# Black-Phoenix/CUDA-SfM

Hardware: AMD Instinct MI355X
Metric: RANSAC E-matrix hypotheses/sec (8-point, fused scoring), inlier-mask parity vs CPU oracle (higher is better)
Workload: dtype f32

## Files before the change

### cuda-sfm_amd/csrc/prefilter_lds.hpp

```cpp
#pragma once
#include "prefilter_record.hpp"

namespace sfm {

constexpr int kPfTileMax = 1024;
constexpr int kPfWaves = 16;
constexpr int kPfRing = 128;

constexpr int kPfERow = 10;
constexpr int kPfPassRows = 32, kPfPairRows = 64;
constexpr int pf_wave_bytes(int rows) { return rows * kPfERow * 4 + rows * 4; }
template <int RULE> struct PfLds {
    static constexpr int kFragsPerBlock = RULE == kPfRuleG ? 3 : 2;
    static constexpr int kBlockBytes = kFragsPerBlock * 64 * 16;
    static constexpr int kFrag = 0;
    static constexpr int kTileMax = kPfTileMax;
    int staged, pts, ring, wave, next, lut, bytes;
    __host__ __device__ explicit PfLds(int tile, int ring_entries = kPfRing, int entry_bytes = 8, int rows = RULE == kPfRuleG ? kPfPassRows : kPfPairRows)
    {
        staged = (tile + 63) & ~63;
        pts = kFrag + (staged / 32) * kBlockBytes;
        ring = pts + staged * 16;
        ring = (ring + ring_entries * entry_bytes - 1) & ~(ring_entries * entry_bytes - 1);
        wave = ring + kPfWaves * ring_entries * entry_bytes;
        next = wave + kPfWaves * pf_wave_bytes(rows);
        lut = next + 16;
        bytes = lut + 32;
    }
};
static_assert(kPfRing * 8 == 1024, "ring slots are addressed with (offset & 1023) | base");

static inline int pf_tile_points(int ld, int tmax)
{
    const int ntiles = (ld + tmax - 1) / tmax;
    const int t = ((ld + ntiles - 1) / ntiles + 31) & ~31;
    return t < 32 ? 32 : t;
}

constexpr unsigned long long kPfSumCountsMin = 1ull << 21;
static inline bool pf_sums_counts_at(unsigned count, int ld, int tile)
{
    return (unsigned long long)count * (unsigned long long)((ld + tile - 1) / tile) >= kPfSumCountsMin;
}

constexpr unsigned long long kPfPairPassesMin = 1ull << 22;
static inline bool pf_pairs_passes_at(unsigned count, int ld, int tile)
{
    return (unsigned long long)count * (unsigned long long)((ld + tile - 1) / tile) >= kPfPairPassesMin;
}

}
```

### cuda-sfm_amd/csrc/prefilter_math.hpp

```cpp
#pragma once
#include "device_math.hpp"

namespace sfm {

constexpr int kPfSlots = 32;
constexpr int kPfSlotsT = 16;
constexpr float kPfRho = 0.125f;
constexpr float kPfFeatScale = 16.0f;
constexpr float kPfPadValue = 256.0f;

struct PfScales { int a; float sigE, sigF, sig2a, inv_sig2a; };

SFM_HD bool prefilter_scales(float thr, PfScales &sc)
{
    if (!(thr >= 1e-9f && thr <= 1e-2f)) return false;
    int e = 0;
    (void)frexpf(1.0f / (32.0f * thr), &e);
    const int a = (e - 1) >> 1;
    sc.a = a;
    sc.sigE = ldexpf(1.0f, a - 4);
    sc.sigF = kPfFeatScale;
    sc.sig2a = ldexpf(1.0f, 2 * a);
    sc.inv_sig2a = ldexpf(1.0f, -2 * a);
    return true;
// ... 357 lines not shown

SFM_HD bool prefilter_band_reject(float nt)
{
    return ((f32_bits(nt) >> 30) & 1u) != 0u;
}

SFM_HD bool prefilter_band_pack_reject(float nt)
{
    return fabsf(nt) >= kPfBandPackSwitch;
}

SFM_HD constexpr uint32_t pf_pack_code(int b)
{
    const int bitpos = 31 - b, odd = bitpos & 1, p = bitpos - odd;
    const int reg = (p % 6 == 4) ? 0 : (p % 6 == 2) ? 1 : 2;
    const int f = (32 * (reg + 3 * odd) + p - 4) / 6;
    const int j = f >> 1, st = f & 1;
    return (uint32_t)((j & 3) + 8 * (j >> 2)) | ((uint32_t)st << 5);
}

SFM_HD constexpr uint32_t pf_pack_code_closed(int b)
{
    const uint32_t f = ((5u * ((uint32_t)b >> 1) + 15u) & 15u) | ((~(uint32_t)b & 1u) << 4);
    return ((f >> 1) & 3u) | (f & 24u) | ((f & 1u) << 5);
}
constexpr bool pf_pack_code_closed_ok()
{
    for (int b = 0; b < 32; ++b)
        if (pf_pack_code_closed(b) != pf_pack_code(b)) return false;
    return true;
}
static_assert(pf_pack_code_closed_ok(), "pf_pack_code_closed: the closed form is not the table's permutation");

SFM_HD constexpr uint32_t pf_pack_field_local(int p)
{
    return (uint32_t)(p % 6 == 4 ? p / 6 : p % 6 == 2 ? p / 6 + 5 : p / 6 + 10);
}
SFM_HD constexpr unsigned long long pf_pack_table()
{
    unsigned long long t = 0ull;
    for (int i = 0; i < 16; ++i) t |= (unsigned long long)pf_pack_field_local(30 - 2 * i) << (4 * i);
    return t;
}
SFM_HD uint32_t pf_pack_field(int b)
{
    constexpr unsigned long long kTable = pf_pack_table();
    const uint32_t local = (uint32_t)(kTable >> (((uint32_t)b << 1) & 60u)) & 15u;
    return local + ((~(uint32_t)b & 1u) << 4);
}

SFM_HD void prefilter_transposed(const float e[9], float et[9])
{
    et[0] = e[0]; et[1] = e[3]; et[2] = e[6];
    et[3] = e[1]; et[4] = e[4]; et[5] = e[7];
    et[6] = e[2]; et[7] = e[5]; et[8] = e[8];
}

SFM_HD uint32_t pf_cell_key_side(int ix, int iy, int side)
{
    const uint32_t k = pf_cell_key(ix, iy);
    return side ? ((k ^ 0x2AAAAAAAu) | 1u) : k;
}

}
```

### cuda-sfm_amd/csrc/ransac_prefilter.hip

```cpp
#include "ransac_device.hpp"
#include "block_ops.hpp"
#include "prefilter_math.hpp"
#include "prefilter_record.hpp"
#include "prefilter_lds.hpp"

namespace sfm {

typedef float f16v __attribute__((ext_vector_type(16)));


__device__ constexpr int kPfESlot[9] = { 2, 6, 1, 3, 5, 7, 0, 4, 8 };
__device__ __forceinline__ uint32_t shift_in_reject(uint32_t rejected, float nt, float G)
{
    return __builtin_amdgcn_alignbit(rejected, __float_as_uint(fmaf(-nt, nt, G)), 31);
}

__device__ __forceinline__ uint32_t scan16(const f16v &nt, const f16v &G)
{
    uint32_t rejected = 0u;
#pragma unroll
    for (int r = 0; r < 16; ++r) rejected = shift_in_reject(rejected, nt[r], G[r]);
    return rejected;
}

// ... 65 lines not shown

template <int RULE>
__device__ __forceinline__ void mfma_step(const PfFrags &a, const PfFrags &b, f16v &G, f16v &nt)
{
    const f16v z = {};
    nt = __builtin_amdgcn_mfma_f32_32x32x16_f16(a.n0, b.n0, z, 0, 0, 0);
    if (RULE == kPfRuleG) G = __builtin_amdgcn_mfma_f32_32x32x16_f16(a.t, b.t, z, 0, 0, 0);
    nt = __builtin_amdgcn_mfma_f32_32x32x16_f16(a.n1, b.n1, nt, 0, 0, 0);
}

#define PF_SCHED_STEP()                                                 \
    do {                                                                \
        if (RULE != kPfRuleG) {                                         \
            __builtin_amdgcn_sched_group_barrier(0x008, 1, 0);          \
            __builtin_amdgcn_sched_group_barrier(0x002, 8, 0);          \
            __builtin_amdgcn_sched_group_barrier(0x008, 1, 0);          \
            __builtin_amdgcn_sched_group_barrier(0x002, 8, 0);          \
        } else {                                                        \
            __builtin_amdgcn_sched_group_barrier(0x008, 1, 0);          \
            __builtin_amdgcn_sched_group_barrier(0x002, 11, 0);         \
            __builtin_amdgcn_sched_group_barrier(0x008, 1, 0);          \
            __builtin_amdgcn_sched_group_barrier(0x002, 11, 0);         \
            __builtin_amdgcn_sched_group_barrier(0x008, 1, 0);          \
            __builtin_amdgcn_sched_group_barrier(0x002, 11, 0);         \
        }                                                               \
    } while (0)

constexpr int kPfVarTickets = 1;
constexpr int kPfVarDrainLocal = 2;
constexpr int kPfVarClosedDecode = 4;
constexpr int kPfVarAnswerEpilogue = 8;
constexpr int kPfVarDrainK1 = 16, kPfVarDrainK7 = 32;
constexpr int kPfVarSinglePass = 64;

constexpr int pf_score_waves_per_simd(int var, int rule, int fl2, int pipe, int wide, int prio)
{
    if (var == 0 && rule == kPfRuleBandTile && !fl2 && !pipe && !wide && !prio) return 4;
    return ((var & kPfVarTickets) == 0 && (rule == kPfRuleBandTile || rule == kPfRuleBandPack) && !fl2 && !pipe && !wide && !prio) ? 5 : 4;
}

template <int W, int VAR = 0, int RULE = kPfRuleBandTile, int FL2 = 0, int PIPE = 0, int WIDE = 0, int PRIO = 0>
__global__ __launch_bounds__(W * 64, pf_score_waves_per_simd(VAR, RULE, FL2, PIPE, WIDE, PRIO))
void ransac_score_prefilter(const float *__restrict__ X0, const float *__restrict__ X1, int ld, int n,
                            const float *__restrict__ Ecand, const PfRecord *__restrict__ recs, uint32_t h0, uint32_t count, float thr,
                            int dynamic, int tile,
                            int *__restrict__ counts, uint32_t *__restrict__ tick,
                            unsigned long long *best_key, unsigned long long *best_key2, unsigned long long *__restrict__ clk,
                            const unsigned long long *__restrict__ bound_word, const uint32_t *__restrict__ tile_boxes)
{
    extern __shared__ __attribute__((aligned(16))) unsigned char smem[];
    const int lane = threadIdx.x & 63;
    const int wave = __builtin_amdgcn_readfirstlane(threadIdx.x >> 6);
    const bool probe = clk && blockIdx.x == 0 && blockIdx.y == 0 && threadIdx.x == 0;
    unsigned long long c0 = 0, w0 = 0;
    if (clk && blockIdx.x == 0 && blockIdx.y == 0 && wave == 0) { c0 = clock64(); w0 = wall_clock64(); }
#if SFM_AB
    const uint32_t trace_blk = blockIdx.y * gridDim.x + blockIdx.x;
    unsigned long long *trace = (clk && trace_blk < (uint32_t)kTraceBlocks) ? clk + 8 + (size_t)trace_blk * kTraceWords : nullptr;
    if (trace && threadIdx.x == 0) {
        trace[0] = wall_clock64();
        trace[2] = ((unsigned long long)__builtin_amdgcn_s_getreg((20 << 0) | (0 << 6) | (31 << 11)) << 32) |
                   (unsigned long long)__builtin_amdgcn_s_getreg((4 << 0) | (0 << 6) | (31 << 11));
        trace[3] = ((unsigned long long)blockIdx.y << 32) | blockIdx.x;
    }
#define PF_PHASE(k) do { if (probe1) clk[k] = wall_clock64() - w0; } while (0)
#else
#define PF_PHASE(k) do { } while (0)
#endif
    const int half = lane >> 5, row = lane & 31;
    uint32_t npass = (count + (uint32_t)kPfGroup - 1u) / (uint32_t)kPfGroup;
    const uint32_t nstatic = gridDim.x * (uint32_t)W;
    using LT = PfLds<RULE>;
    constexpr bool kBand = RULE != kPfRuleG, kTile = RULE == kPfRuleBandTile, kPack = RULE == kPfRuleBandPack || kTile;
    static_assert(!(FL2 && kPack) && !((VAR & kPfVarTickets) && kPack), "the recorded variants were built on the v_alignbit scan");
    constexpr bool kTail9 = kPack && W == 16 && !FL2 && !PIPE && !WIDE && !PRIO && !(VAR & kPfVarTickets);
    static_assert(kTail9 || (VAR & ~kPfVarTickets) == 0, "the pass-tail switches belong to the product's two rules");
    static_assert(!(VAR & kPfVarSinglePass) || (kTile && VAR == kPfVarSinglePass), "single passes: the per-tile rule's summing instance");
    constexpr bool kPair = kTile && kTail9 && VAR == 0;
    constexpr int kRows = kPair ? kPfPairRows : kPfPassRows, kUnit = kRows;
    constexpr int kDrainMore = !kTail9 ? 0 : (VAR & kPfVarDrainK1) ? 1 : (VAR & kPfVarDrainK7) ? 7 : (VAR & kPfVarDrainLocal) ? 3 : 0;
    constexpr bool kDecodeTable = !(kTail9 && (VAR & kPfVarClosedDecode));
    constexpr bool kSumCounts = kTail9 && !(VAR & kPfVarAnswerEpilogue);
    constexpr int kRing = FL2 ? 256 : kPfRing;
    constexpr int kEnt = WIDE ? 16 : 8;
    static_assert(!WIDE || (kPack && !PIPE && !FL2), "wide entries: the packed scan's plain loop only");
    if (kPair) npass = (npass + 1u) >> 1;
    const LT L(tile, kRing, kEnt, kRows);
    float *etab = reinterpret_cast<float *>(smem + L.wave + wave * pf_wave_bytes(kRows));
    int *cnt = reinterpret_cast<int *>(etab + kRows * kPfERow);

    PfFrags afrag = {};
    h8 bfrag_n0 = {}, bfrag_n1 = {};
    uint32_t key0 = 0u;
    float rec_dn = 0.0f, rec_lin = 0.0f;
    float e_row[9] = {};
    auto fetch_pass = [&](uint32_t pass, PfFrags &af, uint32_t &k0, float (&e)[9], float &dn, float &lin) {
        const uint32_t hf = pass * (uint32_t)kUnit;
        const uint32_t h = hf + (uint32_t)min(kPair ? lane : row, (int)min((uint32_t)kUnit, count - hf) - 1);
        if (kTile) {
            const float *src = Ecand + 9 * (size_t)h;
#pragma unroll
            for (int k = 0; k < 9; ++k) e[k] = src[k];
            const uint4 rec = reinterpret_cast<const uint4 *>(recs)[h];
            k0 = rec.x; dn = __uint_as_float(rec.y); lin = __uint_as_float(rec.z);
            return;
        }
        const uint4 *r = reinterpret_cast<const uint4 *>(recs + h) + 2 * half;
        const uint4 r0 = r[0], r1 = r[1];
        if (kBand) pf_band_record_expand(r0, r1, half, af.n0, af.n1, k0);
        else pf_record_expand(r0, r1, half, af.n0, af.n1, af.t, k0);
        if (half == 0) {
            const float *src = Ecand + 9 * (size_t)h;
#pragma unroll
            for (int k = 0; k < 9; ++k) e[k] = src[k];
        }
    };
    auto install_rows = [&](const float (&e)[9]) {
        if (kPair || half == 0) {
            const int r = kPair ? lane : row;
#pragma unroll
            for (int k = 0; k < 9; ++k) etab[kRows * k + r] = e[kPfESlot[k]];
            cnt[r] = 0;
        }
    };
    uint32_t ps = blockIdx.x * (uint32_t)W + (uint32_t)wave;
    bool have = ps < npass;
    if (have) { fetch_pass(ps, afrag, key0, e_row, rec_dn, rec_lin); install_rows(e_row); }

    SFM_PHASE("stage_tile");
    uint32_t *next_idx = reinterpret_cast<uint32_t *>(smem + L.next);
    if (threadIdx.x == 0) *next_idx = (uint32_t)W;
    if (kPack && kDecodeTable && threadIdx.x < 32) smem[L.lut + threadIdx.x] = (unsigned char)pf_pack_code((int)threadIdx.x);
    float pf_B = 0.0f;
    uint32_t bw[8] = {};
    uint32_t bw_lane = 0u;
    if (kTile) {
        pf_B = __uint_as_float((uint32_t)(__hip_atomic_load(reinterpret_cast<const uint32_t *>(bound_word), __ATOMIC_RELAXED, __HIP_MEMORY_SCOPE_AGENT)));
        bw_lane = __hip_atomic_load(tile_boxes + 8 * blockIdx.y + (lane & 7), __ATOMIC_RELAXED, __HIP_MEMORY_SCOPE_AGENT);
    }
    __syncthreads();
    const int tile_first = blockIdx.y * tile;
    for (int t = threadIdx.x; t < L.staged; t += W * 64) {
        const int p = tile_first + t;
        float u = 0.f, v = 0.f, x = 0.f, y = 0.f;
        const bool real = p < n && t < tile;
        if (kTile) {
            if (real) {
                const float4 q4 = reinterpret_cast<const float4 *>(X0)[p];
                u = q4.x; v = q4.y; x = q4.z; y = q4.w;
            }
        } else
        if (real) { u = X0[p]; v = X0[(size_t)ld + p]; x = X1[p]; y = X1[(size_t)ld + p]; }
        _Float16 bn[kPfSlots], bt[kPfSlotsT];
        prefilter_point_slots(u, v, x, y, real, bn, bt);
        reinterpret_cast<float4 *>(smem + L.pts)[t] = real ? make_float4(x, u, y, v) : make_float4(NAN, NAN, NAN, NAN);
        const int pb = t >> 5, col = t & 31;
        unsigned char *blk = smem + LT::kFrag + pb * LT::kBlockBytes;
#pragma unroll
        for (int ks = 0; ks < 2; ++ks)
#pragma unroll
            for (int hh = 0; hh < 2; ++hh) {
                h8 c;
#pragma unroll
                for (int j = 0; j < 8; ++j) c[j] = bn[ks * 16 + hh * 8 + j];
// ... 30 lines not shown
            bfrag_n0 = __builtin_bit_cast(h8, ya); bfrag_n1 = __builtin_bit_cast(h8, yb);
        } else
        pf_tile_operands(e, fl, dn, lin, thr_l, B_l, tbox, half_l, afrag.n0, afrag.n1);
    };
    if (kTile) {
#pragma unroll
        for (int k = 0; k < 8; ++k) bw[k] = (uint32_t)__builtin_amdgcn_readlane((int)bw_lane, k);
        pf_B = uniform(pf_B);
        tbox = pf_box_from_bits(bw, pf_B);
        tbox = PfBox{ uniform(tbox.xlo), uniform(tbox.xhi), uniform(tbox.ylo), uniform(tbox.yhi), uniform(tbox.ulo), uniform(tbox.uhi), uniform(tbox.vlo), uniform(tbox.vhi) };
        if (have) build_operands(e_row, key0, rec_dn, rec_lin);
    }
#if SFM_AB
    if (probe) clk[2] = wall_clock64() - w0;
#endif
    const int npb = (min(tile, ld - tile_first) + 31) >> 5;
    const int npp = (npb + 1) >> 1;
    const float4 *pts = reinterpret_cast<const float4 *>(smem + L.pts);
    lds_cf *etab_l = (lds_cf *)etab;
    lds_i *cnt_l = (lds_i *)cnt;
    lds_cu8 *lut_l = (lds_cu8 *)(smem + L.lut);
    const uint32_t ring_base = (uint32_t)(size_t)(__attribute__((address_space(3))) unsigned char *)(smem + L.ring) + (uint32_t)wave * (uint32_t)(kRing * kEnt);
    uint32_t ring_mask = (uint32_t)(kRing * kEnt - 1);
    asm("" : "+v"(ring_mask));
    auto ring_at = [&](uint32_t index8) {
        return (lds_u2 *)((__attribute__((address_space(3))) unsigned char *)0 + ((index8 & ring_mask) | ring_base));
    };
    auto ring_at16 = [&](uint32_t index16) {
        return (lds_u4 *)((__attribute__((address_space(3))) unsigned char *)0 + ((index16 & ring_mask) | ring_base));
    };
    lds_ch8 *frag_lane = (lds_ch8 *)(smem + LT::kFrag) + lane;
    const ThrBand band = make_band(thr);
    uint32_t passes_done = 0;

    while (have) {
        SFM_PHASE("pass_begin");
        const uint32_t h_first = ps * (uint32_t)kUnit;
        const int nvalid_unit = (int)min((uint32_t)kUnit, count - h_first);
        int nvalid = min(nvalid_unit, kPfGroup), hoff = 0;
        const int nscan = (kPair && nvalid_unit > kPfGroup) ? 2 : 1;
#if SFM_AB
        const bool probe1 = probe && passes_done == 0u;
#endif
        uint32_t ps_next = ps + nstatic;
        if (dynamic) {
            uint32_t got = 0u;
            if (lane == 0) got = atomicAdd(next_idx, 1u);
            got = (uint32_t)__builtin_amdgcn_readfirstlane((int)got);
            ps_next = (got / (uint32_t)W) * nstatic + blockIdx.x * (uint32_t)W + (got % (uint32_t)W);
        }
        const unsigned long long scan_rows = __ballot(key0 != 0u);
        int head = 0, nq = 0;
        auto patch_zero_divisor_rows = [&](int sc) {
            uint32_t todo = kPair ? (uint32_t)(sc ? scan_rows >> 32 : scan_rows) : ((uint32_t)scan_rows | (uint32_t)(scan_rows >> 32));
            uint32_t survive = 0u;
            while (todo) {
                const int r = __builtin_ctz(todo) + hoff;
                todo &= todo - 1u;
                const float se[6] = { etab[6 * kRows + r], etab[2 * kRows + r], etab[r], etab[3 * kRows + r], etab[7 * kRows + r], etab[4 * kRows + r] };
                bool z = false;
                for (int j = 0; j < L.staged / 64; ++j) {
                    const float4 q = pts[j * 64 + lane];
                    z = z || prefilter_zero_divisor(se, q.x, q.z);
                }
                if (__ballot(z) != 0ull) survive |= 1u << (r - hoff);
            }
            if (survive != 0u && ((survive >> row) & 1u)) {
                const h8 zero = {};
                afrag.n0 = zero; afrag.n1 = zero; afrag.t = zero;
                if (half) { afrag.n1[3] = (_Float16)1.0f; afrag.t[7] = (_Float16)0.0009765625f; }
            }
        };

        const uint32_t lane_tag = (uint32_t)(size_t)(lds_cf4 *)pts + (uint32_t)(row * 16) + (uint32_t)(half * 4);
        auto decide_first = [&](uint32_t &rest, uint32_t tag) {
            const int b = __builtin_clz(rest);
            rest &= ~(0x80000000u >> b);
            int hl, sub;
            if (kPack) {
                const uint32_t code = kDecodeTable ? (uint32_t)lut_l[b] : pf_pack_code_closed(b);
                hl = (int)(code & 31u) + (int)(tag & 4u); sub = (int)(code >> 5);
            } else {
                const int r = kBand ? b >> 1 : b & 15;
                sub = kBand ? b & 1 : b >> 4;
                hl = r + (r & 12) + (int)(tag & 4u);
            }
            if (hl < nvalid) {
                const f4v q = *(lds_cf4 *)((__attribute__((address_space(3))) const unsigned char *)0 + ((tag & ~15u) + ((uint32_t)sub << 9)));
                lds_cf *e = etab_l + hl + hoff;
                const v2f p0 = { e[0], e[kRows] }, p1 = { e[2 * kRows], e[3 * kRows] }, p2 = { e[4 * kRows], e[5 * kRows] }, p3 = { e[6 * kRows], e[7 * kRows] };
                const float e8 = e[8 * kRows];
                if (pf_exact_inlier(p0, p1, p2, p3, e8, v2f{ q.x, q.y }, v2f{ q.z, q.w }, band))
                    __hip_atomic_fetch_add(cnt_l + hl + hoff, 1, __ATOMIC_RELAXED, __HIP_MEMORY_SCOPE_WORKGROUP);
            }
        };
        auto flush = [&](int m, auto more_c) {
            constexpr int kMore = decltype(more_c)::value;
            uint32_t rest = 0, tag = 0;
            if (PRIO == 2) __builtin_amdgcn_s_setprio(2);
            if (lane < m) {
                const u2v ent = *ring_at(((uint32_t)head + (uint32_t)lane) * 8u);
                tag = ent.y;
                rest = ent.x;
                decide_first(rest, tag);
                if constexpr (kMore > 0) {
#pragma unroll 1
                    for (int it = 0; it < kMore && rest != 0u; ++it) decide_first(rest, tag);
                }
            }
            const unsigned long long more = __ballot(rest != 0u);
            if (more) {
                const int slot = __builtin_amdgcn_mbcnt_hi((uint32_t)(more >> 32), __builtin_amdgcn_mbcnt_lo((uint32_t)more, 0u));
                if (rest) *ring_at(((uint32_t)(head + nq) + (uint32_t)slot) * 8u) = u2v{ rest, tag };
            }
            head = (head + m) & (kRing - 1);
            nq += __builtin_popcountll(more) - m;
            if (PRIO == 2) __builtin_amdgcn_s_setprio(0);
        };
        constexpr std::integral_constant<int, 0> kInLoop{};
        constexpr std::integral_constant<int, kDrainMore> kDrain{};
        auto flush_w = [&](int m) {
            uint32_t ra = 0, rb = 0, tag = 0;
            if (lane < m) {
                const u4v ent = *ring_at16(((uint32_t)head + (uint32_t)lane) * 16u);
                tag = ent.z;
                const bool second = ent.x == 0u;
// ... 22 lines not shown
        };
        auto flush2 = [&]() {
            const u2v entA = *ring_at(((uint32_t)head + (uint32_t)lane) * 8u), entB = *ring_at(((uint32_t)head + 64u + (uint32_t)lane) * 8u);
            const int bA = __builtin_clz(entA.x), bB = __builtin_clz(entB.x);
            const uint32_t restA = entA.x & ~(0x80000000u >> bA), restB = entB.x & ~(0x80000000u >> bB);
            const int rA = bA >> 1, rB = bB >> 1;
            const int hlA = rA + (rA & 12) + (int)(entA.y & 4u), hlB = rB + (rB & 12) + (int)(entB.y & 4u);
            const int hcA = min(hlA, nvalid - 1), hcB = min(hlB, nvalid - 1);
            const f4v qA = *(lds_cf4 *)((__attribute__((address_space(3))) const unsigned char *)0 + ((entA.y & ~15u) + ((uint32_t)(bA & 1) << 9)));
            const f4v qB = *(lds_cf4 *)((__attribute__((address_space(3))) const unsigned char *)0 + ((entB.y & ~15u) + ((uint32_t)(bB & 1) << 9)));
            lds_cf *eA = etab_l + hcA, *eB = etab_l + hcB;
            const v2f a0 = { eA[0], eA[32] }, a1 = { eA[64], eA[96] }, a2 = { eA[128], eA[160] }, a3 = { eA[192], eA[224] };
            const float a8 = eA[256];
            const v2f b0 = { eB[0], eB[32] }, b1 = { eB[64], eB[96] }, b2 = { eB[128], eB[160] }, b3 = { eB[192], eB[224] };
            const float b8 = eB[256];
            const bool inA = pf_exact_inlier(a0, a1, a2, a3, a8, v2f{ qA.x, qA.y }, v2f{ qA.z, qA.w }, band);
            const bool inB = pf_exact_inlier(b0, b1, b2, b3, b8, v2f{ qB.x, qB.y }, v2f{ qB.z, qB.w }, band);
            if (inA && hlA < nvalid) __hip_atomic_fetch_add(cnt_l + hlA, 1, __ATOMIC_RELAXED, __HIP_MEMORY_SCOPE_WORKGROUP);
            if (inB && hlB < nvalid) __hip_atomic_fetch_add(cnt_l + hlB, 1, __ATOMIC_RELAXED, __HIP_MEMORY_SCOPE_WORKGROUP);
            const unsigned long long moreA = __ballot(restA != 0u), moreB = __ballot(restB != 0u);
            if (moreA | moreB) {
                const int nA = __builtin_popcountll(moreA);
                const int slotA = __builtin_amdgcn_mbcnt_hi((uint32_t)(moreA >> 32), __builtin_amdgcn_mbcnt_lo((uint32_t)moreA, 0u));
                const int slotB = nA + __builtin_amdgcn_mbcnt_hi((uint32_t)(moreB >> 32), __builtin_amdgcn_mbcnt_lo((uint32_t)moreB, 0u));
                if (restA) *ring_at(((uint32_t)(head + nq) + (uint32_t)slotA) * 8u) = u2v{ restA, entA.y };
                if (restB) *ring_at(((uint32_t)(head + nq) + (uint32_t)slotB) * 8u) = u2v{ restB, entB.y };
            }
            head = (head + 128) & (kRing - 1);
            nq += __builtin_popcountll(moreA) + __builtin_popcountll(moreB) - 128;
        };

        for (int sc = 0; ; ++sc) {
        patch_zero_divisor_rows(sc);
        PF_PHASE(3);
        if constexpr (kPack && PIPE) {
        PfFrags fa = load_point_frags<RULE>(frag_lane, 0), fb = load_point_frags<RULE>(frag_lane, 1);
        lds_ch8 *fp = frag_lane + 2 * (LT::kBlockBytes / 16);
        const f16v zero16 = {};
        f16v a0, a1, b0, b1;
        a0 = __builtin_amdgcn_mfma_f32_32x32x16_f16(afrag.n0, fa.n0, zero16, 0, 0, 0);
        a1 = __builtin_amdgcn_mfma_f32_32x32x16_f16(afrag.n0, fb.n0, zero16, 0, 0, 0);
        a0 = __builtin_amdgcn_mfma_f32_32x32x16_f16(afrag.n1, fa.n1, a0, 0, 0, 0);
        a1 = __builtin_amdgcn_mfma_f32_32x32x16_f16(afrag.n1, fb.n1, a1, 0, 0, 0);
        fa = load_point_frags<RULE>(fp, 0);
        fb = load_point_frags<RULE>(fp, 1);
        fp += 2 * (LT::kBlockBytes / 16);
        auto phase = [&](const f16v &c0, const f16v &c1, f16v &m0, f16v &m1, int pp) {
            SFM_PHASE("scan_two_steps");
            __builtin_amdgcn_sched_barrier(0);
            m0 = __builtin_amdgcn_mfma_f32_32x32x16_f16(afrag.n0, fa.n0, zero16, 0, 0, 0);
            __builtin_amdgcn_sched_barrier(0);
            const u6v d = __builtin_amdgcn_cvt_scalef32_2xpk16_bf6_f32(c0, c1, 1.0f);
            __builtin_amdgcn_sched_barrier(0);
            m1 = __builtin_amdgcn_mfma_f32_32x32x16_f16(afrag.n0, fb.n0, zero16, 0, 0, 0);
            __builtin_amdgcn_sched_barrier(0);
            const uint32_t rej32 = pack_reject_bits(d);
            __builtin_amdgcn_sched_barrier(0);
            m0 = __builtin_amdgcn_mfma_f32_32x32x16_f16(afrag.n1, fa.n1, m0, 0, 0, 0);
            __builtin_amdgcn_sched_barrier(0);
            const bool mine = rej32 != 0xFFFFFFFFu;
            const unsigned long long any = __ballot(mine);
            __builtin_amdgcn_sched_barrier(0);
            m1 = __builtin_amdgcn_mfma_f32_32x32x16_f16(afrag.n1, fb.n1, m1, 0, 0, 0);
            __builtin_amdgcn_sched_barrier(0);
            fa = load_point_frags<RULE>(fp, 0);
            fb = load_point_frags<RULE>(fp, 1);
            fp += 2 * (LT::kBlockBytes / 16);
// ... 67 lines not shown
        mfma_step<RULE>(afrag, fa, g0, n0);
        lds_ch8 *fp = frag_lane + 2 * (LT::kBlockBytes / 16);
        for (int pp = 0; pp < npp; ++pp) {
            SFM_PHASE("scan_two_steps");
            fa = load_point_frags<RULE>(fp, 0);
            __builtin_amdgcn_sched_barrier(0);
            mfma_step<RULE>(afrag, fb, g1, n1);
            const uint32_t rej_first = kBand ? scan16_band(n0) : scan16(n0, g0);
            PF_SCHED_STEP();
            __builtin_amdgcn_sched_barrier(0);
            fb = load_point_frags<RULE>(fp, 1);
            fp += 2 * (LT::kBlockBytes / 16);
            __builtin_amdgcn_sched_barrier(0);
            mfma_step<RULE>(afrag, fa, g0, n0);
            const uint32_t rej_second = kBand ? scan16_band(n1) : scan16(n1, g1);
            PF_SCHED_STEP();
            __builtin_amdgcn_sched_barrier(0);
            const uint32_t rej32 = kBand ? (((rej_first << 1) & 0xAAAAAAAAu) | (rej_second & 0x55555555u))
                                                       : ((rej_first << 16) | rej_second);
            const bool mine = rej32 != 0xFFFFFFFFu;
            const unsigned long long any = __ballot(mine);
            SFM_PHASE("append_and_inloop_flush");
            if (any) {
                if (FL2) { while (nq >= 128) flush2(); }
                else
                while (nq >= 64) flush(64, kInLoop);
                const int slot = __builtin_amdgcn_mbcnt_hi((uint32_t)(any >> 32), __builtin_amdgcn_mbcnt_lo((uint32_t)any, 0u));
                if (mine) *ring_at(((uint32_t)(head + nq) + (uint32_t)slot) * 8u) = u2v{ ~rej32, lane_tag + ((uint32_t)pp << 10) };
                nq += __builtin_popcountll(any);
            }
        }
        }
        if (sc + 1 >= nscan) break;
        while (nq > 0) flush(min(nq, 64), kDrain);
        afrag.n0 = bfrag_n0; afrag.n1 = bfrag_n1;
        hoff = kPfGroup; nvalid = nvalid_unit - kPfGroup;
        }
        PF_PHASE(4);
        SFM_PHASE("pass_end_fetch_next");
        const bool have_next = ps_next < npass;
        PfFrags afrag_next = afrag;
        uint32_t key0n = 0u;
        float e_next[9] = {}, dn_next = 0.0f, lin_next = 0.0f;
        if (have_next) fetch_pass(ps_next, afrag_next, key0n, e_next, dn_next, lin_next);
        SFM_PHASE("drain_flush");
        if (FL2) { while (nq >= 128) flush2(); }
        if (WIDE) { while (nq > 0) flush_w(min(nq, 64)); }
        while (nq > 0) flush(min(nq, 64), kDrain);
        SFM_PHASE("epilogue");
        PF_PHASE(7);
        if (VAR & kPfVarTickets) {
        if (lane < nvalid) {
            const int c = cnt[lane];
            if (c) atomicAdd(&counts[h_first + lane], c);
        }
        asm volatile("s_waitcnt vmcnt(0)" ::: "memory");
        uint32_t t = 0;
        if (lane == 0) t = atomicAdd(&tick[ps], 1u);
        t = __builtin_amdgcn_readfirstlane(t);
        if (t == gridDim.y - 1) {
            unsigned long long k = 0;
            if (lane < nvalid) {
                const int c = __hip_atomic_load(&counts[h_first + lane], __ATOMIC_RELAXED, __HIP_MEMORY_SCOPE_AGENT);
                k = pack_key((uint32_t)c, h0 + h_first + (uint32_t)lane);
            }
            k = wave_max(k);
            if (lane == 0 && k) {
// ... 21 lines not shown
        }
        const int nvalid_done = nvalid;
        const uint32_t h_done = h_first;
        if (have_next) {
            if (kTile) build_operands(e_next, key0n, dn_next, lin_next);
            else { afrag = afrag_next; key0 = key0n; }
            install_rows(e_next);
        }
        unsigned long long k = 0;
        if (lane < nvalid_done && (uint32_t)(old >> 32) == gridDim.y - 1u) {
            const uint32_t total = (uint32_t)old + c_mine;
            counts[h_done + lane] = (int)total;
            k = pack_key(total, h0 + h_done + (uint32_t)lane);
        }
        if (__ballot(k != 0ull) != 0ull) {
            k = wave_max(k);
            if (lane == 0 && k > __hip_atomic_load(best_key, __ATOMIC_RELAXED, __HIP_MEMORY_SCOPE_AGENT)) {
                atomicMax(best_key, k);
                if (best_key2) atomicMax(best_key2, k);
            }
        }
        }
        PF_PHASE(5);
        ++passes_done;
        have = have_next;
        if (have_next) {
            ps = ps_next;
            if (VAR & kPfVarTickets) { afrag = afrag_next; key0 = key0n; install_rows(e_next); }
        }
    }
    SFM_PHASE("kernel_end");
    if (probe) { clk[6] = passes_done; clk[0] = clock64() - c0; clk[1] = wall_clock64() - w0; }
#if SFM_AB
    if (trace && lane == 0) {
        const unsigned long long tend = wall_clock64();
        trace[4 + wave] = tend;
        if (wave == 0) trace[1] = tend;
    }
#endif
}

constexpr int kPfBuckets = 1024 + 2;
constexpr int kPfBucketBlock = 256;

__device__ __forceinline__ int pf_bucket_of(const float4 q, float B)
{
    const float big = fmaxf(fmaxf(fabsf(q.x), fabsf(q.y)), fmaxf(fabsf(q.z), fabsf(q.w)));
    if (!(big <= 48.0f) || q.x != q.x || q.y != q.y || q.z != q.z || q.w != q.w) return kPfBuckets - 2;
    return (int)(pf_morton_key(q.x, q.y, -B, B, -B, B) >> 20);
}

__global__ __launch_bounds__(1024)
void pf_bucket_scan_kernel(uint32_t *__restrict__ hist, int nblocks, uint32_t *__restrict__ base, uint32_t *__restrict__ boxes, int nbox_words)
{
    for (int k = threadIdx.x; k < nbox_words; k += blockDim.x) boxes[k] = pf_order_bits(-INFINITY);
    __shared__ uint32_t total[kPfBuckets + 1024];
    for (int b = threadIdx.x; b < kPfBuckets; b += blockDim.x) {
        uint32_t run = 0u;
        for (int k = 0; k < nblocks; ++k) {
            const uint32_t c = hist[(size_t)k * kPfBuckets + b];
            hist[(size_t)k * kPfBuckets + b] = run;
            run += c;
        }
        total[b] = run;
    }
    __syncthreads();
// ... 346 lines not shown
constexpr uint64_t kPfOrderFirstCallPairs = 1ull << 33;
int prefilter_pick_rule(sfm_pair *pair, const sfm_ransac_params &p, uint32_t count)
{
    int rule = pf_rule_switch(p);
    if (rule < 0) {
        const bool ordered = pair->sorted_epoch == pair->bound_epoch && pair->d_pts4s != nullptr;
        const bool first = pair->pf_seen_epoch != pair->bound_epoch;
        rule = (!ordered && first && (uint64_t)count * (uint64_t)pair->ld < kPfOrderFirstCallPairs) ? kPfRuleBandPack : kPfRuleBandTile;
    }
    pair->pf_seen_epoch = pair->bound_epoch;
    pair->pf_rule = rule;
    return rule;
}

bool prefilter_usable(const sfm_pair *pair, const sfm_ransac_params &p, uint32_t count)
{
    PfScales sc;
    return pair->state.unit_z && pair->state.have_bound && count >= 16384u && (uint64_t)count * (uint64_t)pair->ld >= (1ull << 27) && prefilter_scales(p.threshold, sc);
}

static int pf_tile_of(const sfm_pair *pair, const sfm_ransac_params &p)
{
    if (SFM_SW(p, 1) == 7 && pair->pf_rule == kPfRuleBand) return pf_tile_points(pair->ld, 1536);
    return pf_tile_points(pair->ld, kPfTileMax);
}

int prefilter_tile_points(const sfm_pair *pair, const sfm_ransac_params &p) { return pf_tile_of(pair, p); }

static int pf_tail_var(const sfm_pair *pair, const sfm_ransac_params &p, uint32_t count)
{
    const bool large = pf_sums_counts_at(count, pair->ld, pf_tile_of(pair, p));
    if (SFM_SW(p, 1) == 19) return 0;
    if (SFM_SW(p, 1) == 20) return pair->pf_rule == kPfRuleBandTile ? kPfVarSinglePass : 0;
    if (pair->pf_rule == kPfRuleBandTile && SFM_SW(p, 1) == 16) return kPfVarDrainK1;
    if (pair->pf_rule == kPfRuleBandTile && SFM_SW(p, 1) == 17) return kPfVarDrainK7;
    int var = 0;
    const bool lab = SFM_SW(p, 3) >= 8 && SFM_SW(p, 3) < 16;
    if (lab && (SFM_SW(p, 3) & 1)) var |= kPfVarDrainLocal;
    if (lab && (SFM_SW(p, 3) & 2)) var |= kPfVarClosedDecode;
    const bool sum = (lab && (SFM_SW(p, 3) & 4)) ? false : (large || (SFM_SW(p, 1) >= 16 && SFM_SW(p, 1) <= 18));
    if (!sum) var |= kPfVarAnswerEpilogue;
    if (var == 0 && pair->pf_rule == kPfRuleBandTile && !pf_pairs_passes_at(count, pair->ld, pf_tile_of(pair, p))) var = kPfVarSinglePass;
    return var;
}

bool prefilter_sums_counts(const sfm_pair *pair, const sfm_ransac_params &p, uint32_t count)
{
    const bool product_rule = pair->pf_rule == kPfRuleBandTile || pair->pf_rule == kPfRuleBandPack;
    const bool variant = SFM_SW(p, 1) == 5 || (SFM_SW(p, 1) >= 11 && SFM_SW(p, 1) <= 15);
    return product_rule && !variant && !(pf_tail_var(pair, p, count) & kPfVarAnswerEpilogue);
}

int launch_score_prefilter(sfm_pair *pair, ShardSlot &s, hipStream_t stream, const sfm_ransac_params &p, uint32_t h0, uint32_t count, unsigned long long *key2)
{
    sfm_ctx *ctx = pair->ctx;
    PfScales sc;
    if (!prefilter_scales(p.threshold, sc)) { set_error("threshold %g outside the pre-filter's range", (double)p.threshold); return SFM_E_INVALID; }
    const int waves = (SFM_SW(p, 1) == 5 || SFM_SW(p, 1) == 12) ? 12 : kPfWaves;
    const int tile = pf_tile_of(pair, p);
    const int ntiles = (pair->ld + tile - 1) / tile;
    const uint32_t npass = (count + (uint32_t)kPfGroup - 1u) / (uint32_t)kPfGroup;
    const int rule = pair->pf_rule;
    const int tail_var = pf_tail_var(pair, p, count);
    const bool wide = rule == kPfRuleBandTile && SFM_SW(p, 1) == 13;
    const bool paired_units = rule == kPfRuleBandTile && tail_var == 0 && waves == kPfWaves && !wide && SFM_SW(p, 1) != 14 && SFM_SW(p, 1) != 15;
    const uint32_t nunits = paired_units ? (npass + 1u) / 2u : npass;
    const uint32_t iters = (nunits + (uint32_t)waves - 1) / (uint32_t)waves;
    uint32_t cols = (uint32_t)ctx->num_cus / (uint32_t)ntiles;
    if (SFM_SW(p, 2) > 0) cols = (uint32_t)SFM_SW(p, 2);
    if (cols > iters) cols = iters;
    if (cols < 1) cols = 1;
    const int dynamic = SFM_SW(p, 1) == 2 ? 0 : 1;
    const int var = SFM_SW(p, 3) >= 16 ? SFM_SW(p, 3) - 16 : 0;
    const bool fl2 = rule == kPfRuleBand && waves == kPfWaves && SFM_SW(p, 1) == 9;
    const int lds_bytes = wide ? PfLds<kPfRuleBand>(tile, kPfRing, 16, kPfPassRows).bytes : fl2 ? PfLds<kPfRuleBand>(tile, 256, 8, kPfPassRows).bytes
                        : rule != kPfRuleG ? PfLds<kPfRuleBand>(tile, kPfRing, 8, paired_units ? kPfPairRows : kPfPassRows).bytes : PfLds<kPfRuleG>(tile).bytes;
    if (lds_bytes > 160 * 1024) { set_error("pre-filter tile of %d points needs %d bytes of LDS", tile, lds_bytes); return SFM_E_INVALID; }
    auto launch = [&](auto kernel) -> int {
        const int rc_lds = allow_big_lds(ctx, reinterpret_cast<const void *>(kernel));
        if (rc_lds != SFM_OK) return rc_lds;
        const float *x0 = rule == kPfRuleBandTile ? reinterpret_cast<const float *>(pair->d_pts4s) : pair->d_X[0];
        hipLaunchKernelGGL(kernel, dim3(cols, ntiles), dim3(waves * 64), lds_bytes, stream,
                           x0, pair->d_X[1], pair->ld, pair->n, s.Ecand, reinterpret_cast<const PfRecord *>(s.pf), h0, count, p.threshold,
                           dynamic, tile, s.counts, s.tick, s.key, key2, pair->d_clk, pair->d_bound, pair->d_tile_boxes);
        return SFM_OK;
    };
    int rcl;
#if SFM_AB
    if (rule == kPfRuleG && waves == 12) rcl = launch(&ransac_score_prefilter<12, 0, kPfRuleG>);
    else if (rule == kPfRuleG && var == 1) rcl = launch(&ransac_score_prefilter<16, 1, kPfRuleG>);
    else if (rule == kPfRuleG) rcl = launch(&ransac_score_prefilter<16, 0, kPfRuleG>);
    else if (waves == 12) rcl = launch(&ransac_score_prefilter<12, 0, kPfRuleBand>);
    else if (fl2) rcl = launch(&ransac_score_prefilter<16, 0, kPfRuleBand, 1>);
    else if (rule == kPfRuleBand) rcl = launch(&ransac_score_prefilter<16, 0, kPfRuleBand>);
    else if (SFM_SW(p, 1) == 11) rcl = launch(&ransac_score_prefilter<16, 0, kPfRuleBandPack, 0, 1>);
    else if (SFM_SW(p, 1) == 12) rcl = launch(&ransac_score_prefilter<12, 0, kPfRuleBandPack, 0, 1>);
    else if (wide) rcl = launch(&ransac_score_prefilter<16, 0, kPfRuleBandTile, 0, 0, 1>);
    else if (rule == kPfRuleBandTile && SFM_SW(p, 1) == 14) rcl = launch(&ransac_score_prefilter<16, 0, kPfRuleBandTile, 0, 0, 0, 1>);
    else if (rule == kPfRuleBandTile && SFM_SW(p, 1) == 15) rcl = launch(&ransac_score_prefilter<16, 0, kPfRuleBandTile, 0, 0, 0, 2>);
    else if (tail_var != 0 && tail_var != kPfVarAnswerEpilogue && tail_var != kPfVarSinglePass) {
        rcl = SFM_E_INVALID;
#define PF_TAIL_CASE(V) case V: rcl = rule == kPfRuleBandPack ? launch(&ransac_score_prefilter<16, V, kPfRuleBandPack>) : launch(&ransac_score_prefilter<16, V, kPfRuleBandTile>); break
        switch (tail_var) {
        PF_TAIL_CASE(2); PF_TAIL_CASE(4); PF_TAIL_CASE(6); PF_TAIL_CASE(10); PF_TAIL_CASE(12); PF_TAIL_CASE(14);
        case kPfVarDrainK1: rcl = launch(&ransac_score_prefilter<16, kPfVarDrainK1, kPfRuleBandTile>); break;
        case kPfVarDrainK7: rcl = launch(&ransac_score_prefilter<16, kPfVarDrainK7, kPfRuleBandTile>); break;
        default: set_error("pass-tail switches %d: no such instance", tail_var); break;
        }
#undef PF_TAIL_CASE
    }
    else
#endif
    if (tail_var & kPfVarAnswerEpilogue) rcl = rule == kPfRuleBandPack ? launch(&ransac_score_prefilter<16, kPfVarAnswerEpilogue, kPfRuleBandPack>)
                                                                       : launch(&ransac_score_prefilter<16, kPfVarAnswerEpilogue, kPfRuleBandTile>);
    else if (rule == kPfRuleBandPack) rcl = launch(&ransac_score_prefilter<16, 0, kPfRuleBandPack>);
    else if (tail_var == kPfVarSinglePass) rcl = launch(&ransac_score_prefilter<16, kPfVarSinglePass, kPfRuleBandTile>);
    else rcl = launch(&ransac_score_prefilter<16, 0, kPfRuleBandTile>);
    (void)var; (void)fl2; (void)wide; (void)tail_var;
    if (rcl != SFM_OK) return rcl;
    SFM_HIP_TRY(hipGetLastError());
    pair->last_grid = (int)cols * ntiles; pair->last_block = waves * 64; pair->last_lds = lds_bytes;
    return SFM_OK;
}

}
```

### profiles/phase_probe.py

```python
import json
import os
import sys

sys.path.insert(0, os.path.dirname(os.path.dirname(os.path.abspath(__file__))))
import numpy as np
import torch
import cuda_sfm_amd_ab as S
from cuda_sfm_amd_ab import synth

dev = torch.device("cuda", 0)
ctx = S.Context(0, torch.cuda.current_stream().cuda_stream)
n = 4096
scene = synth.two_view_scene(n)
d_sift = torch.from_numpy(scene["sift"].view(np.uint8).reshape(n, 576)).to(dev)
pair = S.ImagePair(ctx, scene["K"], scene["Kinv"], 2, n)
pair.fillXU(d_sift)
label = sys.argv[1] if len(sys.argv) > 1 else None
r1, r3, samples = (int(sys.argv[k]) if len(sys.argv) > k else d for k, d in ((2, 0), (3, 0), (4, 1)))
cases = ((1048576, 0),) * samples if label else ((131072, 0), (131072, 64), (262144, 0), (1048576, 0), (1048576, 64))
for H, cols in cases:
    p = S.default_params(n, num_hypotheses=H, seed=3, kernel=S.KERNEL_PREFILTER)
    p.reserved[1], p.reserved[2], p.reserved[3] = r1, cols, r3
    for _ in range(10):
        pair.estimateE(p)
    ctx.kernel_timing(True) if hasattr(ctx, "kernel_timing") else None
    pair.estimateE(p)
    t = pair.last_phases()
    us = lambda k: round(t[k] / 100.0, 2)
    tag = {"build": label, "reserved": [0, r1, cols, r3], "drain_us": round((t[7] - t[4]) / 100.0, 2), "epilogue_us": round((t[5] - t[7]) / 100.0, 2)} if label else {}
    print(json.dumps({**tag, "hypotheses": H, "grid": pair.last_launch()["grid"], "block0_lifetime_us": us(1), "tile_staged_us": us(2), "first_pass_prepared_us": us(3),
                      "first_block_scanned_us": us(4), "ring_drained_us": us(7), "first_pass_done_us": us(5), "passes_of_wave0": t[6],
                      "shader_mhz": round(100.0 * t[0] / max(t[1], 1))}), flush=True)
```

Before: 2.806 billion.

## Carry queued ring entries across paired scans instead of draining between them

In the default paired-unit kernel, the ring of candidate entries is no longer flushed between the first and second scan. Each entry is tagged with a scan bit, and a larger 128-byte LDS lookup table maps packed code plus tag to the hypothesis row, so both scans' rows decode from one table. The old drain-between-scans behaviour stays available as a switchable variant for A/B comparison. This removes a serialising drain at the scan boundary, at the cost of a bigger LUT, extra tag bits, and possibly more entries held in the ring at once.

```diff
diff --git a/cuda-sfm_amd/csrc/prefilter_lds.hpp b/cuda-sfm_amd/csrc/prefilter_lds.hpp
--- a/cuda-sfm_amd/csrc/prefilter_lds.hpp
+++ b/cuda-sfm_amd/csrc/prefilter_lds.hpp
@@ -25,7 +25,7 @@
         wave = ring + kPfWaves * ring_entries * entry_bytes;
         next = wave + kPfWaves * pf_wave_bytes(rows);
         lut = next + 16;
-        bytes = lut + 32;
+        bytes = lut + kPfRingLutBytes;
     }
 };
 static_assert(kPfRing * 8 == 1024, "ring slots are addressed with (offset & 1023) | base");
diff --git a/cuda-sfm_amd/csrc/prefilter_math.hpp b/cuda-sfm_amd/csrc/prefilter_math.hpp
--- a/cuda-sfm_amd/csrc/prefilter_math.hpp
+++ b/cuda-sfm_amd/csrc/prefilter_math.hpp
@@ -413,6 +413,19 @@
 }
 static_assert(pf_pack_code_closed_ok(), "pf_pack_code_closed: the closed form is not the table's permutation");
 
+constexpr uint32_t kPfTagHalf = 4u, kPfTagScan = 8u;
+SFM_HD constexpr int pf_ring_row(uint32_t code, uint32_t tag)
+{
+    return (int)(code & 31u) + (int)(tag & kPfTagHalf) + (int)((tag & kPfTagScan) << 2);
+}
+constexpr int kPfRingLutBytes = 128;
+SFM_HD constexpr uint32_t pf_ring_lut_index(int b, uint32_t tag) { return (uint32_t)b | ((tag & (kPfTagHalf | kPfTagScan)) << 3); }
+SFM_HD constexpr uint32_t pf_ring_lut_entry(uint32_t index)
+{
+    const uint32_t code = pf_pack_code((int)(index & 31u));
+    return (uint32_t)pf_ring_row(code, (index >> 5) << 2) | ((code >> 5) << 6);
+}
+
 SFM_HD constexpr uint32_t pf_pack_field_local(int p)
 {
     return (uint32_t)(p % 6 == 4 ? p / 6 : p % 6 == 2 ? p / 6 + 5 : p / 6 + 10);
diff --git a/cuda-sfm_amd/csrc/ransac_prefilter.hip b/cuda-sfm_amd/csrc/ransac_prefilter.hip
--- a/cuda-sfm_amd/csrc/ransac_prefilter.hip
+++ b/cuda-sfm_amd/csrc/ransac_prefilter.hip
@@ -121,10 +121,11 @@
 constexpr int kPfVarAnswerEpilogue = 8;
 constexpr int kPfVarDrainK1 = 16, kPfVarDrainK7 = 32;
 constexpr int kPfVarSinglePass = 64;
+constexpr int kPfVarPairDrain = 128;
 
 constexpr int pf_score_waves_per_simd(int var, int rule, int fl2, int pipe, int wide, int prio)
 {
-    if (var == 0 && rule == kPfRuleBandTile && !fl2 && !pipe && !wide && !prio) return 4;
+    if ((var == 0 || var == kPfVarPairDrain) && rule == kPfRuleBandTile && !fl2 && !pipe && !wide && !prio) return 4;
     return ((var & kPfVarTickets) == 0 && (rule == kPfRuleBandTile || rule == kPfRuleBandPack) && !fl2 && !pipe && !wide && !prio) ? 5 : 4;
 }
 
@@ -165,7 +166,9 @@
     constexpr bool kTail9 = kPack && W == 16 && !FL2 && !PIPE && !WIDE && !PRIO && !(VAR & kPfVarTickets);
     static_assert(kTail9 || (VAR & ~kPfVarTickets) == 0, "the pass-tail switches belong to the product's two rules");
     static_assert(!(VAR & kPfVarSinglePass) || (kTile && VAR == kPfVarSinglePass), "single passes: the per-tile rule's summing instance");
-    constexpr bool kPair = kTile && kTail9 && VAR == 0;
+    static_assert(!(VAR & kPfVarPairDrain) || (kTile && VAR == kPfVarPairDrain), "paired passes drained between the scans: the per-tile rule's summing instance");
+    constexpr bool kPair = kTile && kTail9 && (VAR == 0 || VAR == kPfVarPairDrain);
+    constexpr bool kCarry = kPair && VAR == 0;
     constexpr int kRows = kPair ? kPfPairRows : kPfPassRows, kUnit = kRows;
     constexpr int kDrainMore = !kTail9 ? 0 : (VAR & kPfVarDrainK1) ? 1 : (VAR & kPfVarDrainK7) ? 7 : (VAR & kPfVarDrainLocal) ? 3 : 0;
     constexpr bool kDecodeTable = !(kTail9 && (VAR & kPfVarClosedDecode));
@@ -219,6 +222,9 @@
     SFM_PHASE("stage_tile");
     uint32_t *next_idx = reinterpret_cast<uint32_t *>(smem + L.next);
     if (threadIdx.x == 0) *next_idx = (uint32_t)W;
+    if constexpr (kCarry) {
+        if (threadIdx.x < kPfRingLutBytes) smem[L.lut + threadIdx.x] = (unsigned char)pf_ring_lut_entry(threadIdx.x);
+    } else
     if (kPack && kDecodeTable && threadIdx.x < 32) smem[L.lut + threadIdx.x] = (unsigned char)pf_pack_code((int)threadIdx.x);
     float pf_B = 0.0f;
     uint32_t bw[8] = {};
@@ -315,6 +321,9 @@
     lds_ch8 *frag_lane = (lds_ch8 *)(smem + LT::kFrag) + lane;
     const ThrBand band = make_band(thr);
     uint32_t passes_done = 0;
+#if SFM_AB
+    uint32_t carried = 0;
+#endif
 
     while (have) {
         SFM_PHASE("pass_begin");
@@ -324,6 +333,7 @@
         const int nscan = (kPair && nvalid_unit > kPfGroup) ? 2 : 1;
 #if SFM_AB
         const bool probe1 = probe && passes_done == 0u;
+        unsigned long long w_scan_end = 0;
 #endif
         uint32_t ps_next = ps + nstatic;
         if (dynamic) {
@@ -355,12 +365,15 @@
             }
         };
 
-        const uint32_t lane_tag = (uint32_t)(size_t)(lds_cf4 *)pts + (uint32_t)(row * 16) + (uint32_t)(half * 4);
+        uint32_t lane_tag = (uint32_t)(size_t)(lds_cf4 *)pts + (uint32_t)(row * 16) + (uint32_t)(half * 4);
         auto decide_first = [&](uint32_t &rest, uint32_t tag) {
             const int b = __builtin_clz(rest);
             rest &= ~(0x80000000u >> b);
             int hl, sub;
-            if (kPack) {
+            if constexpr (kCarry) {
+                const uint32_t code = (uint32_t)lut_l[pf_ring_lut_index(b, tag)];
+                hl = (int)(code & 63u); sub = (int)(code >> 6);
+            } else if (kPack) {
                 const uint32_t code = kDecodeTable ? (uint32_t)lut_l[b] : pf_pack_code_closed(b);
                 hl = (int)(code & 31u) + (int)(tag & 4u); sub = (int)(code >> 5);
             } else {
@@ -368,13 +381,14 @@
                 sub = kBand ? b & 1 : b >> 4;
                 hl = r + (r & 12) + (int)(tag & 4u);
             }
-            if (hl < nvalid) {
+            const int row_end = kCarry ? nvalid_unit : nvalid, row_first = kCarry ? 0 : hoff;
+            if (hl < row_end) {
                 const f4v q = *(lds_cf4 *)((__attribute__((address_space(3))) const unsigned char *)0 + ((tag & ~15u) + ((uint32_t)sub << 9)));
-                lds_cf *e = etab_l + hl + hoff;
+                lds_cf *e = etab_l + hl + row_first;
                 const v2f p0 = { e[0], e[kRows] }, p1 = { e[2 * kRows], e[3 * kRows] }, p2 = { e[4 * kRows], e[5 * kRows] }, p3 = { e[6 * kRows], e[7 * kRows] };
                 const float e8 = e[8 * kRows];
                 if (pf_exact_inlier(p0, p1, p2, p3, e8, v2f{ q.x, q.y }, v2f{ q.z, q.w }, band))
-                    __hip_atomic_fetch_add(cnt_l + hl + hoff, 1, __ATOMIC_RELAXED, __HIP_MEMORY_SCOPE_WORKGROUP);
+                    __hip_atomic_fetch_add(cnt_l + hl + row_first, 1, __ATOMIC_RELAXED, __HIP_MEMORY_SCOPE_WORKGROUP);
             }
         };
         auto flush = [&](int m, auto more_c) {
@@ -463,7 +477,10 @@
 
         for (int sc = 0; ; ++sc) {
         patch_zero_divisor_rows(sc);
-        PF_PHASE(3);
+#if SFM_AB
+        if (sc == 0) PF_PHASE(3);
+        else if (probe1) reinterpret_cast<uint32_t *>(clk + 3)[1] = (uint32_t)(wall_clock64() - w_scan_end);
+#endif
         if constexpr (kPack && PIPE) {
         PfFrags fa = load_point_frags<RULE>(frag_lane, 0), fb = load_point_frags<RULE>(frag_lane, 1);
         lds_ch8 *fp = frag_lane + 2 * (LT::kBlockBytes / 16);
@@ -597,7 +614,14 @@
         }
         }
         if (sc + 1 >= nscan) break;
-        while (nq > 0) flush(min(nq, 64), kDrain);
+#if SFM_AB
+        if (probe1) w_scan_end = wall_clock64();
+#endif
+        if constexpr (kCarry) lane_tag |= kPfTagScan;
+        else while (nq > 0) flush(min(nq, 64), kDrain);
+#if SFM_AB
+        carried += (uint32_t)nq;
+#endif
         afrag.n0 = bfrag_n0; afrag.n1 = bfrag_n1;
         hoff = kPfGroup; nvalid = nvalid_unit - kPfGroup;
         }
@@ -685,6 +709,7 @@
     SFM_PHASE("kernel_end");
     if (probe) { clk[6] = passes_done; clk[0] = clock64() - c0; clk[1] = wall_clock64() - w0; }
 #if SFM_AB
+    if (probe) clk[6] |= (unsigned long long)carried << 32;
     if (trace && lane == 0) {
         const unsigned long long tend = wall_clock64();
         trace[4 + wave] = tend;
@@ -1097,6 +1122,7 @@
     const bool large = pf_sums_counts_at(count, pair->ld, pf_tile_of(pair, p));
     if (SFM_SW(p, 1) == 19) return 0;
     if (SFM_SW(p, 1) == 20) return pair->pf_rule == kPfRuleBandTile ? kPfVarSinglePass : 0;
+    if (SFM_SW(p, 1) == 21) return pair->pf_rule == kPfRuleBandTile ? kPfVarPairDrain : 0;
     if (pair->pf_rule == kPfRuleBandTile && SFM_SW(p, 1) == 16) return kPfVarDrainK1;
     if (pair->pf_rule == kPfRuleBandTile && SFM_SW(p, 1) == 17) return kPfVarDrainK7;
     int var = 0;
@@ -1128,7 +1154,7 @@
     const int rule = pair->pf_rule;
     const int tail_var = pf_tail_var(pair, p, count);
     const bool wide = rule == kPfRuleBandTile && SFM_SW(p, 1) == 13;
-    const bool paired_units = rule == kPfRuleBandTile && tail_var == 0 && waves == kPfWaves && !wide && SFM_SW(p, 1) != 14 && SFM_SW(p, 1) != 15;
+    const bool paired_units = rule == kPfRuleBandTile && (tail_var == 0 || tail_var == kPfVarPairDrain) && waves == kPfWaves && !wide && SFM_SW(p, 1) != 14 && SFM_SW(p, 1) != 15;
     const uint32_t nunits = paired_units ? (npass + 1u) / 2u : npass;
     const uint32_t iters = (nunits + (uint32_t)waves - 1) / (uint32_t)waves;
     uint32_t cols = (uint32_t)ctx->num_cus / (uint32_t)ntiles;
@@ -1170,6 +1196,7 @@
         PF_TAIL_CASE(2); PF_TAIL_CASE(4); PF_TAIL_CASE(6); PF_TAIL_CASE(10); PF_TAIL_CASE(12); PF_TAIL_CASE(14);
         case kPfVarDrainK1: rcl = launch(&ransac_score_prefilter<16, kPfVarDrainK1, kPfRuleBandTile>); break;
         case kPfVarDrainK7: rcl = launch(&ransac_score_prefilter<16, kPfVarDrainK7, kPfRuleBandTile>); break;
+        case kPfVarPairDrain: rcl = launch(&ransac_score_prefilter<16, kPfVarPairDrain, kPfRuleBandTile>); break;
         default: set_error("pass-tail switches %d: no such instance", tail_var); break;
         }
 #undef PF_TAIL_CASE
diff --git a/profiles/kernel_text_hashes.py b/profiles/kernel_text_hashes.py
--- /dev/null
+++ b/profiles/kernel_text_hashes.py
@@ -0,0 +1,27 @@
+import hashlib
+import os
+import re
+import subprocess
+import sys
+
+ROOT = os.path.dirname(os.path.dirname(os.path.abspath(__file__)))
+src = sys.argv[1]
+want = sys.argv[2] if len(sys.argv) > 2 else ""
+flags = ["--offload-arch=gfx950", "-O3", "-std=c++17", "-ffp-contract=off", "-fhip-fp32-correctly-rounded-divide-sqrt", "-DOCML_BASIC_ROUNDED_OPERATIONS",
+         "-fPIC", "-fvisibility=hidden", "-Wno-unused-function", "-Wno-pass-failed", "--cuda-device-only", "-S"]
+text = subprocess.run([os.environ.get("HIPCC", "/opt/rocm/bin/hipcc")] + flags + [src, "-o", "-"], cwd=ROOT, check=True, capture_output=True, text=True).stdout
+name, body = None, []
+for line in text.splitlines():
+    m = re.match(r"^(_Z\w+):", line)
+    if m and name is None:
+        name, body = m.group(1), []
+        continue
+    if name is None:
+        continue
+    code = line.split(";")[0].strip()
+    if code and not code.startswith("."):
+        body.append(re.sub(r"\.LBB\d+_", ".LBB_", code))
+    if code.startswith(".Lfunc_end"):
+        if want in name:
+            print(hashlib.sha256("\n".join(body).encode()).hexdigest()[:16], len(body), name)
+        name = None
diff --git a/profiles/phase_probe.py b/profiles/phase_probe.py
--- a/profiles/phase_probe.py
+++ b/profiles/phase_probe.py
@@ -25,9 +25,11 @@
         pair.estimateE(p)
     ctx.kernel_timing(True) if hasattr(ctx, "kernel_timing") else None
     pair.estimateE(p)
-    t = pair.last_phases()
+    t = [int(v) for v in pair.last_phases()]
+    boundary_ticks, held = t[3] >> 32, t[6] >> 32
+    t[3] &= 0xFFFFFFFF; t[6] &= 0xFFFFFFFF
     us = lambda k: round(t[k] / 100.0, 2)
     tag = {"build": label, "reserved": [0, r1, cols, r3], "drain_us": round((t[7] - t[4]) / 100.0, 2), "epilogue_us": round((t[5] - t[7]) / 100.0, 2)} if label else {}
     print(json.dumps({**tag, "hypotheses": H, "grid": pair.last_launch()["grid"], "block0_lifetime_us": us(1), "tile_staged_us": us(2), "first_pass_prepared_us": us(3),
-                      "first_block_scanned_us": us(4), "ring_drained_us": us(7), "first_pass_done_us": us(5), "passes_of_wave0": t[6],
+                      "first_block_scanned_us": us(4), "ring_drained_us": us(7), "first_pass_done_us": us(5), "passes_of_wave0": t[6], "scan_boundary_us": round(boundary_ticks / 100.0, 2), "entries_held_at_second_scans": held,
                       "shader_mhz": round(100.0 * t[0] / max(t[1], 1))}), flush=True)
diff --git a/profiles/pipelined_switch_ab.py b/profiles/pipelined_switch_ab.py
--- /dev/null
+++ b/profiles/pipelined_switch_ab.py
@@ -0,0 +1,52 @@
+import json
+import os
+import subprocess
+import sys
+import time
+
+ROOT = os.path.dirname(os.path.dirname(os.path.abspath(__file__)))
+
+if sys.argv[1] == "run":
+    sys.path.insert(0, ROOT)
+    import numpy as np
+    import torch
+    import cuda_sfm_amd_ab as S
+    from cuda_sfm_amd_ab import synth
+    H, sw = int(sys.argv[2]), int(sys.argv[3])
+    dev = torch.device("cuda", 0)
+    n = 4096
+    scene = synth.two_view_scene(n)
+    d_sift = torch.from_numpy(scene["sift"].view(np.uint8).reshape(n, 576)).to(dev)
+    ctx = S.Context(0, torch.cuda.current_stream().cuda_stream)
+    ctx.own_stream()
+    pair = S.ImagePair(ctx, scene["K"], scene["Kinv"], 2, n)
+    pair.fillXU(d_sift)
+    p = S.default_params(n, num_hypotheses=H, kernel=S.KERNEL_PREFILTER)
+    p.reserved[1] = sw
+    for _ in range(20):
+        pair.estimateE_pipelined(p)
+    pair.flush(); ctx.synchronize(); torch.cuda.synchronize()
+    steps = 200
+    t0 = time.perf_counter()
+    for _ in range(steps):
+        pair.estimateE_pipelined(p)
+    pair.flush(); ctx.synchronize(); torch.cuda.synchronize()
+    dt = (time.perf_counter() - t0) / steps
+    launch = pair.last_launch()
+    print(json.dumps({"hypotheses": H, "reserved1": sw, "ms_per_step": dt * 1e3, "lds_bytes": launch["lds_bytes"], "grid": launch["grid"], "best": list(pair.get_best())}))
+    sys.exit(0)
+
+H, switches = int(sys.argv[1]), (int(sys.argv[2]), int(sys.argv[3]))
+reps = int(sys.argv[4]) if len(sys.argv) > 4 else 5
+out = open(sys.argv[5], "w") if len(sys.argv) > 5 else None
+for rep in range(reps):
+    for sw in switches:
+        r = subprocess.run(["timeout", "-k", "10", "120", sys.executable, os.path.abspath(__file__), "run", str(H), str(sw)], cwd=ROOT, capture_output=True, text=True)
+        lines = [ln for ln in r.stdout.splitlines() if ln.startswith("{")]
+        if r.returncode != 0 or not lines:
+            print("FAILED", sw, r.returncode, r.stdout[-1500:], r.stderr[-3000:], flush=True)
+            sys.exit(1)
+        msg = json.dumps({"rep": rep, **json.loads(lines[-1])})
+        print(msg, flush=True)
+        if out:
+            out.write(msg + "\n"); out.flush()
```

New measurement: 2.850 billion (median of 6 runs). 1.5% higher.
